# NVIDIA/k8s-operator-libs

Measured on AMD Instinct MI355X. Metric: 8-node rolling-upgrade wall-clock, lower is better.
Workload: dtype fp32; 1 GPU; model=amdgpu-driver-rolling-upgrade, nodes_per_cluster=8, maxParallelUpgrades=2, maxUnavailable=50%, drain=True, podDeletion=True, gpu_pods_per_node=2, gpu_validation=True, converging_reconcile=True, mode=inplace, global_batch=8, parallelism=dp1 (one independent simulated 8-node cluster per rank)

## Files before the change

### k8s_operator_libs_amd/core/cache.py

```python

from __future__ import annotations

import threading
import time
from typing import Dict, List, Optional, Tuple

from . import meta
from .client import Client
from .errors import NotFoundError
from .meta import K8sObject


class _Informer:
    BACKOFF_BASE = 0.1
    BACKOFF_MAX = 5.0

    USE_WATCH_LIST = True

    USE_DRAIN_ON_READ = True

    def __init__(self, delegate: Client, api_version: str, kind: str,
                 sync_delay: float = 0.0) -> None:
        self.api_version = api_version
        self.kind = kind
# ... 277 lines not shown
                self._informers[key] = inf
                inf.start()
        inf.wait_sync()
        return inf

    def wait_for_resource_version(self, api_version: str, kind: str,
                                  name: str, namespace: str, rv: str,
                                  timeout: float = 10.0) -> bool:
        return self._informer_for(api_version, kind).wait_for_rv(
            name, namespace, rv, timeout
        )

    def wait_for_cache_sync(self, timeout: float = 10.0) -> bool:
        with self._lock:
            informers = list(self._informers.values())
        return all(inf.wait_sync(timeout) for inf in informers)

    def stop(self) -> None:
        with self._lock:
            informers = list(self._informers.values())
            self._informers.clear()
        for inf in informers:
            inf.stop()


    def get(self, api_version, kind, name, namespace=""):
        return self._informer_for(api_version, kind).get(name, namespace)

    def list(self, api_version, kind, namespace=None, label_selector="", field_selector=""):
        return self._informer_for(api_version, kind).list(
            namespace, label_selector, field_selector
        )


    def create(self, obj):
        return self._delegate.create(obj)

    def update(self, obj):
        return self._delegate.update(obj)

    def patch(self, api_version, kind, name, patch, namespace=""):
        return self._delegate.patch(api_version, kind, name, patch, namespace)

    def delete(self, api_version, kind, name, namespace="", grace_period_seconds=None):
        try:
            self._delegate.delete(api_version, kind, name, namespace,
                                  grace_period_seconds=grace_period_seconds)
        except TypeError:
            self._delegate.delete(api_version, kind, name, namespace)

    def evict_pod(self, name, namespace):
        self._delegate.evict_pod(name, namespace)

    def patch_status(self, api_version, kind, name, status, namespace=""):
        return self._delegate.patch_status(api_version, kind, name, status,
                                           namespace)

    def watch(self, api_version, kind, namespace=None, resource_version=None,
              label_selector=""):
        return self._delegate.watch(
            api_version, kind, namespace=namespace,
            resource_version=resource_version, label_selector=label_selector,
        )

    def list_with_meta(self, api_version, kind, namespace=None,
                       label_selector="", field_selector=""):
        return self._delegate.list_with_meta(
            api_version, kind, namespace=namespace,
            label_selector=label_selector, field_selector=field_selector,
        )
```

### k8s_operator_libs_amd/core/client.py

```python

from __future__ import annotations

import abc
from typing import List, Optional

from .fakecluster import FakeCluster, Watch
from .meta import K8sObject


class Client(abc.ABC):

    @abc.abstractmethod
    def get(self, api_version: str, kind: str, name: str, namespace: str = "") -> K8sObject: ...

    @abc.abstractmethod
    def list(
        self,
        api_version: str,
        kind: str,
        namespace: Optional[str] = None,
        label_selector: str = "",
        field_selector: str = "",
    ) -> List[K8sObject]: ...

    @abc.abstractmethod
    def create(self, obj: K8sObject) -> K8sObject: ...

    @abc.abstractmethod
    def update(self, obj: K8sObject) -> K8sObject: ...

    @abc.abstractmethod
    def patch(
        self, api_version: str, kind: str, name: str, patch: K8sObject, namespace: str = ""
    ) -> K8sObject: ...

    @abc.abstractmethod
    def delete(self, api_version: str, kind: str, name: str, namespace: str = "") -> None:
        """Delete an object.  Implementations may accept a
        ``grace_period_seconds`` keyword (pod graceful-deletion override);
        in-memory substrates delete immediately and ignore it."""

    @abc.abstractmethod
    def evict_pod(self, name: str, namespace: str) -> None: ...

    def watch(
        self,
        api_version: str,
        kind: str,
        namespace: Optional[str] = None,
        resource_version: Optional[str] = None,
        label_selector: str = "",
    ) -> Watch:
        raise NotImplementedError("this client does not support watches")

    def list_with_meta(
        self,
        api_version: str,
        kind: str,
        namespace: Optional[str] = None,
        label_selector: str = "",
# ... 99 lines not shown
```

### k8s_operator_libs_amd/core/restclient.py

```python

from __future__ import annotations

import collections
import http.client as _http_client
import json
import os
from typing import Any, Dict, Optional

import httpx

from ..native import load_wire as _load_wire
from . import meta
from .client import Client
from .errors import (
    AlreadyExistsError,
    ApiError,
    BadRequestError,
    ConflictError,
    NotFoundError,
)

SA_DIR = "/var/run/secrets/kubernetes.io/serviceaccount"

_KIND_INFO = {
    ("v1", "Node"): ("nodes", False),
    ("v1", "Pod"): ("pods", True),
    ("v1", "Event"): ("events", True),
    ("v1", "Namespace"): ("namespaces", False),
    ("apps/v1", "DaemonSet"): ("daemonsets", True),
    ("apps/v1", "ControllerRevision"): ("controllerrevisions", True),
    ("apiextensions.k8s.io/v1", "CustomResourceDefinition"): (
        "customresourcedefinitions", False),
    ("maintenance.amd.com/v1alpha1", "NodeMaintenance"): ("nodemaintenances", True),
    ("coordination.k8s.io/v1", "Lease"): ("leases", True),
}


def _lower_plural(kind: str) -> str:
    k = kind.lower()
    if k.endswith(("ss", "x", "z", "ch", "sh")):
        return k + "es"
    if k.endswith("s"):
        return k
    if k.endswith("y") and len(k) > 1 and k[-2] not in "aeiou":
        return k[:-1] + "ies"
    return k + "s"


def _pool_max_idle() -> int:
    from ..upgrade.common_manager import CommonUpgradeManager
    from ..upgrade.drain_manager import DrainManager
    from ..upgrade.pod_manager import PodManager

    return (1 + PodManager.MAX_CONCURRENT_NODE_WORKERS
            + DrainManager.MAX_CONCURRENT_NODE_WORKERS
            + CommonUpgradeManager.MAX_PARALLEL_NODE_OPS)


class RestClient(Client):
    USE_POOL = True

    def __init__(
        self,
        base_url: str,
        token: Optional[str] = None,
        verify: Any = True,
        timeout: float = 30.0,
        extra_kinds: Optional[Dict[tuple, tuple]] = None,
        retries: int = 3,
    ) -> None:
        self.base_url = base_url.rstrip("/")
        headers = {"Content-Type": "application/json"}
        if token:
            headers["Authorization"] = f"Bearer {token}"
        self._headers = dict(headers)
        self._timeout = timeout
        self._http = httpx.Client(
            base_url=self.base_url, headers=headers, verify=verify, timeout=timeout
        )
        self._fast_netloc = None
        self._wire = None
        self._pool = None
        if self.base_url.startswith("http://"):
            import urllib.parse

            parsed = urllib.parse.urlsplit(self.base_url)
            self._fast_netloc = (parsed.hostname, parsed.port or 80)
            self._fast_local = __import__("threading").local()
            self._wire = _load_wire()
            self._wire_heads: Dict[tuple, bytes] = {}
            if self._wire is not None and hasattr(self._wire, "Pool"):
                self._pool = self._wire.Pool(
                    *self._fast_netloc, max_idle=_pool_max_idle(),
                    connect_timeout=timeout)
        self._kinds = dict(_KIND_INFO)
        if extra_kinds:
            self._kinds.update(extra_kinds)
        self._retries = retries


    def _wire_head(self, headers=None) -> bytes:
        key = tuple(sorted(headers.items())) if headers else ()
        head = self._wire_heads.get(key)
        if head is None:
            host, port = self._fast_netloc
            if ":" in host:
                host = f"[{host}]"
            hdrs = {"Host": host if port == 80 else f"{host}:{port}",
                    "Accept-Encoding": "identity"}
            hdrs.update(self._headers)
            if headers:
                hdrs.update(headers)
            head = "".join(f"{k}: {v}\r\n" for k, v in hdrs.items()).encode(
# ... 275 lines not shown
            md = body.get("metadata") or {}
            if rv is None:
                rv = md.get("resourceVersion")
            items.extend(body.get("items", []))
            cont = md.get("continue")
            if not cont:
                return items, rv
            params["continue"] = cont

    def create(self, obj):
        api_version, kind = meta.api_version(obj), meta.kind(obj)
        path = self._collection_path(api_version, kind, meta.namespace(obj))
        resp = self._request("POST", path, content=json.dumps(obj))
        self._raise_for(resp)
        return resp.json()

    def update(self, obj):
        api_version, kind = meta.api_version(obj), meta.kind(obj)
        path = self._object_path(api_version, kind, meta.name(obj), meta.namespace(obj))
        resp = self._request("PUT", path, content=json.dumps(obj))
        self._raise_for(resp)
        return resp.json()

    def patch(self, api_version, kind, name, patch, namespace=""):
        path = self._object_path(api_version, kind, name, namespace)
        resp = self._request(
            "PATCH", path, content=json.dumps(patch),
            headers={"Content-Type": "application/merge-patch+json"},
        )
        self._raise_for(resp)
        return resp.json()

    def delete(self, api_version, kind, name, namespace="", grace_period_seconds=None):
        kw = {}
        if grace_period_seconds is not None:
            kw["content"] = json.dumps({
                "apiVersion": "v1", "kind": "DeleteOptions",
                "gracePeriodSeconds": int(grace_period_seconds),
            })
        resp = self._request(
            "DELETE", self._object_path(api_version, kind, name, namespace), **kw
        )
        self._raise_for(resp)

    def patch_status(self, api_version, kind, name, status, namespace=""):
        path = self._object_path(api_version, kind, name, namespace) + "/status"
        resp = self._request(
            "PATCH", path, content=json.dumps({"status": status}),
            headers={"Content-Type": "application/merge-patch+json"},
        )
        self._raise_for(resp)
        return resp.json()

    def evict_pod(self, name, namespace):
        path = self._object_path("v1", "Pod", name, namespace) + "/eviction"
        body = {
            "apiVersion": "policy/v1",
            "kind": "Eviction",
            "metadata": {"name": name, "namespace": namespace},
        }
        resp = self._request("POST", path, content=json.dumps(body))
        self._raise_for(resp)

    def watch(self, api_version: str, kind: str, namespace=None,
              resource_version=None, label_selector="", field_selector="",
              send_initial_events=False):
        return _HttpWatch(self, api_version, kind, namespace=namespace,
                          resource_version=resource_version,
                          label_selector=label_selector,
                          field_selector=field_selector,
                          send_initial_events=send_initial_events)


    def discover_resource(self, api_version: str, plural: str) -> bool:
        prefix = f"/api/{api_version}" if "/" not in api_version else f"/apis/{api_version}"
        resp = self._request("GET", prefix)
        if resp.status_code != 200:
            return False
        for res in resp.json().get("resources", []):
            if res.get("name") == plural:
                return True
        return False

    def register_kind(self, api_version: str, kind: str, plural: str, namespaced: bool) -> None:
        self._kinds[(api_version, kind)] = (plural, namespaced)

    def close(self) -> None:
        self._http.close()
        if self._fast_netloc is not None:
            conn = getattr(self._fast_local, "conn", None)
            if conn is not None:
                try:
                    conn.close()
                except Exception:
                    pass
                self._fast_local.conn = None
            self._wire_drop(getattr(self._fast_local, "sock", None))
            pool, self._pool = self._pool, None
            if pool is not None:
                pool.close()


class _PoolClosed(Exception):
    """The client was closed while a request was on its way to the pool."""


class _FastResponse:

    __slots__ = ("status_code", "_data")

    def __init__(self, status_code: int, data: bytes) -> None:
        self.status_code = status_code
        self._data = data

    def json(self):
# ... 309 lines not shown
```

### k8s_operator_libs_amd/native/build.py

```python

from __future__ import annotations

import os
import subprocess
import sysconfig

PKG_DIR = os.path.dirname(os.path.abspath(__file__))
SOURCE = os.path.join(PKG_DIR, "gpu_validator.hip")
OUTPUT = os.path.join(PKG_DIR, "_gpu_validator.so")
JSONOPS_SOURCE = os.path.join(PKG_DIR, "jsonops.cpp")
JSONOPS_OUTPUT = os.path.join(PKG_DIR, "_jsonops.so")
WIRE_SOURCES = (
    os.path.join(PKG_DIR, "wire.cpp"),
    os.path.join(PKG_DIR, "wire_core.hpp"),
    os.path.join(PKG_DIR, "wire_pool.hpp"),
    os.path.join(PKG_DIR, "wire_stream.hpp"),
)
WIRE_OUTPUT = os.path.join(PKG_DIR, "_wire.so")

HIPCC = os.environ.get("HIPCC", "/opt/rocm/bin/hipcc")
CXX = os.environ.get("CXX", "g++")


def validator_sources() -> list:
    wire = {os.path.basename(p) for p in WIRE_SOURCES}
    return [SOURCE] + sorted(
        os.path.join(PKG_DIR, name) for name in os.listdir(PKG_DIR)
        if name.endswith(".hpp") and name not in wire)


def is_built() -> bool:
    return os.path.exists(OUTPUT) and all(
        os.path.getmtime(OUTPUT) >= os.path.getmtime(src)
        for src in validator_sources())


def build_jsonops(force: bool = False, verbose: bool = False) -> str:
    if (
        not force
        and os.path.exists(JSONOPS_OUTPUT)
        and os.path.getmtime(JSONOPS_OUTPUT) >= os.path.getmtime(JSONOPS_SOURCE)
    ):
        return JSONOPS_OUTPUT
    cmd = [
        CXX, "-O3", "-std=c++17", "-fPIC", "-shared",
        f"-I{sysconfig.get_paths()['include']}",
        JSONOPS_SOURCE, "-o", JSONOPS_OUTPUT,
    ]
    if verbose:
        print(" ".join(cmd))
    subprocess.run(cmd, check=True, capture_output=not verbose)
    return JSONOPS_OUTPUT


def build_wire(force: bool = False, verbose: bool = False) -> str:
    if (
        not force
        and os.path.exists(WIRE_OUTPUT)
        and all(os.path.getmtime(WIRE_OUTPUT) >= os.path.getmtime(src)
                for src in WIRE_SOURCES)
    ):
        return WIRE_OUTPUT
    cmd = [
        CXX, "-O3", "-std=c++17", "-fPIC", "-shared", "-pthread",
        f"-I{sysconfig.get_paths()['include']}",
        WIRE_SOURCES[0], "-o", WIRE_OUTPUT,
    ]
# ... 36 lines not shown
```

### k8s_operator_libs_amd/native/wire.cpp

```cpp

#define PY_SSIZE_T_CLEAN
#include <Python.h>

#include <atomic>
#include <cerrno>
#include <chrono>
#include <memory>
#include <mutex>
#include <new>
#include <string>
#include <system_error>
#include <thread>
#include <vector>

#include <fcntl.h>
#include <poll.h>
#include <sys/socket.h>
#include <sys/types.h>
#include <unistd.h>

#include "wire_core.hpp"
#include "wire_pool.hpp"
#include "wire_stream.hpp"

namespace {

constexpr size_t kRecvBuf = 64 * 1024;

using Clock = std::chrono::steady_clock;

struct Deadline {
  bool infinite;
  Clock::time_point at;

  explicit Deadline(double timeout_s) : infinite(timeout_s < 0) {
    if (!infinite)
      at = Clock::now() + std::chrono::duration_cast<Clock::duration>(
                              std::chrono::duration<double>(timeout_s));
  }

  int remaining_ms() const {
    if (infinite) return -1;
    auto left = std::chrono::duration_cast<std::chrono::microseconds>(
                    at - Clock::now()).count();
    if (left <= 0) return 0;
    long long ms = (left + 999) / 1000;
    return ms > 0x7fffffff ? 0x7fffffff : int(ms);
  }
};

bool parse_timeout(PyObject* obj, double* out) {
  if (obj == nullptr || obj == Py_None) {
    *out = -1.0;
    return true;
  }
  double v = PyFloat_AsDouble(obj);
  if (v == -1.0 && PyErr_Occurred()) return false;
  *out = v < 0 ? 0.0 : v;
  return true;
}

enum IoResult { kIoOk = 0, kIoTimeout = 1, kIoError = 2, kIoSignal = 3 };

IoResult wait_fd(int fd, short events, const Deadline& dl) {
  for (;;) {
    int ms = dl.remaining_ms();
    struct pollfd p = {fd, events, 0};
    int rc, err;
    Py_BEGIN_ALLOW_THREADS
    rc = poll(&p, 1, ms);
    err = errno;
    Py_END_ALLOW_THREADS
    if (rc > 0) return kIoOk;
    if (rc == 0) {
// ... 73 lines not shown
  return kIoOk;
}

PyObject* raise_wire_error(int st) {
  PyErr_SetString(PyExc_ValueError, wire::status_message(st));
  return nullptr;
}

PyObject* raise_timeout() {
  PyErr_SetString(PyExc_TimeoutError, "timed out");
  return nullptr;
}

bool as_buffer(PyObject* obj, const char** p, Py_ssize_t* n, bool* present) {
  *present = true;
  if (obj == Py_None) {
    *p = "";
    *n = 0;
    *present = false;
    return true;
  }
  if (PyBytes_Check(obj)) {
    *p = PyBytes_AS_STRING(obj);
    *n = PyBytes_GET_SIZE(obj);
    return true;
  }
  if (PyUnicode_Check(obj)) {
    *p = PyUnicode_AsUTF8AndSize(obj, n);
    return *p != nullptr;
  }
  PyErr_SetString(PyExc_TypeError, "body must be bytes, str or None");
  return false;
}


PyObject* py_exchange(PyObject* , PyObject* args) {
  int fd;
  const char *method, *path, *head;
  Py_ssize_t method_len, path_len, head_len;
  PyObject *body_obj, *timeout_obj = Py_None;
  if (!PyArg_ParseTuple(args, "is#s#y#O|O", &fd, &method, &method_len, &path,
                        &path_len, &head, &head_len, &body_obj, &timeout_obj))
    return nullptr;
  const char* body;
  Py_ssize_t body_len;
  bool has_body;
  if (!as_buffer(body_obj, &body, &body_len, &has_body)) return nullptr;
  double timeout_s;
  if (!parse_timeout(timeout_obj, &timeout_s)) return nullptr;
  Deadline dl(timeout_s);

  std::string method_s(method, size_t(method_len));
  bool is_head = method_s == "HEAD";
  bool wants_length = has_body || method_s == "POST" || method_s == "PUT" ||
                      method_s == "PATCH";

  std::string req;
  req.reserve(size_t(method_len + path_len + head_len + body_len) + 64);
  req.append(method_s).append(" ").append(path, size_t(path_len));
  req.append(" HTTP/1.1\r\n").append(head, size_t(head_len));
  if (wants_length)
    req.append("Content-Length: ").append(std::to_string(body_len)).append("\r\n");
  req.append("\r\n").append(body, size_t(body_len));

  IoResult io = send_all(fd, req.data(), req.size(), dl);
  if (io == kIoTimeout) return raise_timeout();
  if (io != kIoOk) return nullptr;

  wire::ResponseReader reader(is_head);
  char buf[kRecvBuf];

  while (!reader.done()) {
    size_t got = 0;
    io = recv_some(fd, buf, sizeof buf, dl, &got);
    if (io == kIoTimeout) return raise_timeout();
    if (io != kIoOk) return nullptr;
    if (got == 0) {
      if (reader.peer_closed()) break;
      bool got_any = reader.started();
      PyErr_SetString(got_any ? PyExc_ConnectionError
                              : PyExc_ConnectionResetError,
                      got_any ? "peer closed the connection mid-response"
                              : "peer closed the connection without a response");
      return nullptr;
    }
    int st = reader.feed(buf, got);
    if (st < 0) return raise_wire_error(st);
  }

  const std::string& out = reader.body();
  PyObject* body_bytes =
      PyBytes_FromStringAndSize(out.data(), Py_ssize_t(out.size()));
  if (!body_bytes) return nullptr;
  PyObject* res = Py_BuildValue("(iNO)", reader.status(), body_bytes,
                                reader.reusable() ? Py_True : Py_False);
  return res;
}


PyObject* py_parse_request_head(PyObject* , PyObject* arg) {
  Py_buffer view;
  if (PyObject_GetBuffer(arg, &view, PyBUF_SIMPLE) < 0) return nullptr;
  wire::HeadParser hp(wire::HeadParser::kRequest);
  size_t used = 0;
  int st = hp.feed(static_cast<const char*>(view.buf), size_t(view.len), &used);
  PyBuffer_Release(&view);
  if (st < 0) return raise_wire_error(st);
  if (st == wire::kNeedMore) Py_RETURN_NONE;
  PyObject* length;
  if (hp.has_content_length) {
    length = PyLong_FromSize_t(hp.content_length);
    if (!length) return nullptr;
  } else {
    length = Py_None;
    Py_INCREF(length);
  }
// ... 783 lines not shown
  switch (lease.error) {
    case wire::Pool::kOk:
      return Py_BuildValue("(iO)", lease.fd,
                           lease.reused ? Py_True : Py_False);
    case wire::Pool::kClosed:
      PyErr_SetString(PyExc_RuntimeError, "Pool is closed");
      return nullptr;
    case wire::Pool::kResolve: {
      PyObject* gaierror = nullptr;
      PyObject* mod = PyImport_ImportModule("socket");
      if (mod != nullptr) {
        gaierror = PyObject_GetAttrString(mod, "gaierror");
        Py_DECREF(mod);
      }
      if (gaierror == nullptr) return nullptr;
      PyObject* val = Py_BuildValue("(is)", lease.code, gai_strerror(lease.code));
      if (val != nullptr) {
        PyErr_SetObject(gaierror, val);
        Py_DECREF(val);
      }
      Py_DECREF(gaierror);
      return nullptr;
    }
    case wire::Pool::kTimeout:
      return raise_timeout();
    case wire::Pool::kInterrupted:
      return nullptr;
    default:
      errno = lease.code;
      return PyErr_SetFromErrno(PyExc_OSError);
  }
}

PyObject* pool_checkout(PoolObject* self, PyObject* args) {
  try {
    return pool_checkout_impl(self, args);
  } catch (const std::bad_alloc&) {
    return PyErr_NoMemory();
  }
}

PyObject* pool_checkin(PoolObject* self, PyObject* args) {
  int fd, reusable;
  if (!PyArg_ParseTuple(args, "ip", &fd, &reusable)) return nullptr;
  if (!pool_enter(self)) return nullptr;
  try {
    self->pool->checkin(fd, reusable != 0);
  } catch (const std::bad_alloc&) {
    close(fd);
  }
  Py_RETURN_NONE;
}

PyObject* pool_close(PoolObject* self, PyObject*) {
  if (!pool_enter(self)) return nullptr;
  self->pool->close();
  Py_RETURN_NONE;
}

PyObject* pool_stats(PoolObject* self, PyObject*) {
  if (!pool_enter(self)) return nullptr;
  wire::PoolStats st = self->pool->stats();
  return Py_BuildValue("{s:K,s:K,s:K,s:n}", "dials",
                       static_cast<unsigned long long>(st.dials), "reuses",
                       static_cast<unsigned long long>(st.reuses),
                       "stale_discards",
                       static_cast<unsigned long long>(st.stale_discards),
                       "idle", Py_ssize_t(st.idle));
}

PyObject* pool_get_max_idle(PoolObject* self, void*) {
  if (!pool_enter(self)) return nullptr;
  return PyLong_FromSize_t(self->pool->max_idle());
}

PyObject* pool_get_closed(PoolObject* self, void*) {
  if (!pool_enter(self)) return nullptr;
  return PyBool_FromLong(self->pool->closed());
}

PyMethodDef pool_methods[] = {
    {"checkout", reinterpret_cast<PyCFunction>(pool_checkout), METH_VARARGS,
     "checkout(fresh=False) -> (fd, reused).  The most recently used idle "
     "connection that is still quiet (reused=True), else (or with fresh) a "
     "new one, dialled with the GIL released.  The fd stays the pool's: pass it to exchange() and "
     "give it back with checkin(), exactly once, never close it.  OSError "
     "(TimeoutError, socket.gaierror) when the dial fails; RuntimeError "
     "once the pool is closed."},
    {"checkin", reinterpret_cast<PyCFunction>(pool_checkin), METH_VARARGS,
     "checkin(fd, reusable).  Give a checked-out fd back.  It is kept for "
     "the next checkout() only when reusable is true (the response was "
     "complete and exchange() said reusable), the pool is open and fewer "
     "than max_idle are idle; otherwise the pool closes it."},
    {"close", reinterpret_cast<PyCFunction>(pool_close), METH_NOARGS,
     "close().  Close the idle connections; one checked out now is closed "
     "when it comes back.  checkout() raises from here on."},
    {"stats", reinterpret_cast<PyCFunction>(pool_stats), METH_NOARGS,
     "stats() -> {'dials', 'reuses', 'stale_discards', 'idle'}."},
    {nullptr, nullptr, 0, nullptr},
};

PyGetSetDef pool_getset[] = {
    {"max_idle", reinterpret_cast<getter>(pool_get_max_idle), nullptr,
     "most connections kept idle", nullptr},
    {"closed", reinterpret_cast<getter>(pool_get_closed), nullptr,
     "True after close()", nullptr},
    {nullptr, nullptr, nullptr, nullptr, nullptr},
};

PyTypeObject PoolType = {
    PyVarObject_HEAD_INIT(nullptr, 0)
    "_wire.Pool",
    sizeof(PoolObject),
};


PyObject* py_exchange_guarded(PyObject* self, PyObject* args) {
  try {
    return py_exchange(self, args);
  } catch (const std::bad_alloc&) {
    return PyErr_NoMemory();
  }
}

PyObject* py_parse_request_head_guarded(PyObject* self, PyObject* arg) {
  try {
    return py_parse_request_head(self, arg);
  } catch (const std::bad_alloc&) {
    return PyErr_NoMemory();
  }
}

PyMethodDef wire_methods[] = {
    {"exchange", py_exchange_guarded, METH_VARARGS,
     "exchange(fd, method, path, header_bytes, body, timeout=None) -> "
     "(status, body_bytes, reusable).  One HTTP/1.1 request/response on a "
     "connected socket: the request goes out in a single send; the response "
     "is read with Content-Length, chunked or read-to-EOF framing.  "
     "reusable is False when the connection must not carry another request."},
    {"parse_request_head", py_parse_request_head_guarded, METH_O,
     "parse_request_head(data) -> None | (method, target, minor_version, "
     "content_length | None, chunked, keep_alive, head_size).  None while "
     "the head is incomplete; ValueError when it is malformed."},
    {nullptr, nullptr, 0, nullptr},
};

// ... 93 lines not shown
```

### k8s_operator_libs_amd/upgrade/drain.py

```python

from __future__ import annotations

import logging
import time
from dataclasses import dataclass, field
from typing import Callable, List, Optional

from ..api.upgrade.v1alpha1 import DrainSpec
from ..core import meta
from ..core.client import Client
from ..core.errors import ApiError, NotFoundError
from . import consts

logger = logging.getLogger(__name__)

MIRROR_POD_ANNOTATION = "kubernetes.io/config.mirror"

PodFilter = Callable[[dict], bool]


@dataclass
class PodDeleteList:

    pods: List[dict] = field(default_factory=list)
# ... 49 lines not shown
    node_name: str,
    *,
    force: bool = False,
    delete_emptydir_data: bool = False,
    ignore_daemonsets: bool = True,
    pod_selector: str = "",
    additional_filter: Optional[PodFilter] = None,
) -> PodDeleteList:
    pods = client.list_pods(
        label_selector=pod_selector,
        field_selector=consts.NODE_NAME_FIELD_SELECTOR_FMT.format(node_name),
    )
    out = PodDeleteList()
    for pod in pods:
        pname = f"{meta.namespace(pod)}/{meta.name(pod)}"
        if _is_terminating(pod):
            out.skipped.append(pod)
            continue
        if additional_filter is not None and not additional_filter(pod):
            out.skipped.append(pod)
            continue
        if _is_mirror_pod(pod):
            out.skipped.append(pod)
            out.warnings.append(f"skipping mirror pod {pname}")
            continue
        if _is_daemonset_pod(pod):
            if ignore_daemonsets:
                out.skipped.append(pod)
                out.warnings.append(f"ignoring DaemonSet-managed pod {pname}")
                continue
            out.errors.append(f"cannot delete DaemonSet-managed pod {pname}")
            continue
        if _is_finished(pod):
            out.pods.append(pod)
            continue
        if not _has_controller(pod) and not force:
            out.errors.append(
                f"cannot delete pod not managed by a controller (use force): {pname}"
            )
            continue
        if _uses_emptydir(pod) and not delete_emptydir_data:
            out.errors.append(
                f"cannot delete pod with emptyDir volume (use deleteEmptyDir): {pname}"
            )
            continue
        out.pods.append(pod)
    return out


class DrainError(Exception):
    pass


def delete_or_evict_pods(
    client: Client,
    pods: List[dict],
    *,
    use_eviction: bool = True,
    timeout_seconds: float = 300,
) -> None:
    deadline = time.monotonic() + max(timeout_seconds, 0.001)

    def try_evict(pod) -> bool:
        try:
            if use_eviction:
                client.evict_pod(meta.name(pod), meta.namespace(pod))
            else:
                client.delete_pod(meta.name(pod), meta.namespace(pod))
            return True
        except NotFoundError:
            return True
        except ApiError as exc:
            if exc.code == 429:
                return False
            raise

    blocked = [pod for pod in pods if not try_evict(pod)]
    interval = 0.001
    remaining = list(pods)
    while remaining:
        blocked = [pod for pod in blocked if not try_evict(pod)]
        still_there = []
        for pod in remaining:
            try:
                live = client.get("v1", "Pod", meta.name(pod), meta.namespace(pod))
            except NotFoundError:
                continue
            if meta.uid(live) == meta.uid(pod):
                still_there.append(pod)
        remaining = still_there
        if not remaining:
            return
        if time.monotonic() >= deadline:
            names = [f"{meta.namespace(p)}/{meta.name(p)}" for p in remaining]
            if blocked:
                names = [f"{n} (PDB-blocked)" if any(
                    meta.name(b) == n.split("/")[-1] for b in blocked) else n
                    for n in names]
            raise DrainError(f"timed out waiting for pods to terminate: {names}")
        time.sleep(interval)
        interval = min(interval * 2, 0.5)


def drain_node(client: Client, node_name: str, spec: DrainSpec) -> None:
    plist = get_pods_for_deletion(
        client,
        node_name,
        force=spec.force,
        delete_emptydir_data=spec.delete_emptydir_data,
        ignore_daemonsets=True,
        pod_selector=spec.pod_selector,
    )
    if plist.errors:
        raise DrainError("; ".join(plist.errors))
    for warning in plist.warnings:
        logger.debug("drain %s: %s", node_name, warning)
    delete_or_evict_pods(
        client, plist.pods, use_eviction=True, timeout_seconds=spec.timeout_seconds
    )
```

### k8s_operator_libs_amd/upgrade/pod_manager.py

```python

from __future__ import annotations

import logging
import threading
import time
from dataclasses import dataclass, field
from typing import Callable, List, Optional

from ..api.upgrade.v1alpha1 import PodDeletionSpec, WaitForCompletionSpec
from ..core import meta
from ..core.client import Client
from ..core.events import EVENT_TYPE_NORMAL, EVENT_TYPE_WARNING, log_event, log_eventf
from ..core.meta import K8sObject
from . import consts, util
from .drain import delete_or_evict_pods, get_pods_for_deletion
from .node_state_provider import NodeUpgradeStateProvider

logger = logging.getLogger(__name__)

class StaleClusterViewError(RuntimeError):
    """The client's view is missing objects that must exist (e.g. a managed
    DaemonSet with no ControllerRevisions): with an informer-backed client
    this is a transient staleness window, not a cluster defect.  Callers
    treat it like any reconcile error — requeue (upgrade_state.go:128-131
    pattern)."""


POD_CONTROLLER_REVISION_HASH_LABEL = "controller-revision-hash"

PodDeletionFilter = Callable[[K8sObject], bool]


@dataclass
class PodManagerConfig:

    nodes: List[K8sObject] = field(default_factory=list)
    deletion_spec: Optional[PodDeletionSpec] = None
    wait_for_completion_spec: Optional[WaitForCompletionSpec] = None
    drain_enabled: bool = False


class PodManager:
    def __init__(
        self,
        client: Client,
        node_state_provider: NodeUpgradeStateProvider,
        pod_deletion_filter: Optional[PodDeletionFilter] = None,
        event_recorder: Optional[object] = None,
    ) -> None:
        self._client = client
        self._provider = node_state_provider
        self._filter = pod_deletion_filter
        self._recorder = event_recorder
        self._nodes_in_progress = util.StringSet()
        self._workers: List[threading.Thread] = []
        self._workers_lock = threading.Lock()
        self._worker_slots = threading.Semaphore(self.MAX_CONCURRENT_NODE_WORKERS)
        self._ds_hash_cache: dict = {}


    def get_pod_controller_revision_hash(self, pod: K8sObject) -> str:
        hash_ = meta.get_label(pod, POD_CONTROLLER_REVISION_HASH_LABEL)
        if not hash_:
            raise ValueError(
                f"pod {meta.name(pod)} has no {POD_CONTROLLER_REVISION_HASH_LABEL} label"
            )
        return hash_

    def get_daemonset_controller_revision_hash(self, daemonset: K8sObject) -> str:
        cache_key = (meta.namespace(daemonset), meta.name(daemonset),
                     meta.resource_version(daemonset))
        cached = self._ds_hash_cache.get(cache_key)
        if cached is not None:
            return cached
        selector = daemonset.get("spec", {}).get("selector", {}).get("matchLabels", {})
        label_selector = ",".join(f"{k}={v}" for k, v in sorted(selector.items()))
        revisions = self._client.list_controller_revisions(
            namespace=meta.namespace(daemonset), label_selector=label_selector
        )
        if not revisions:
            raise StaleClusterViewError(
                f"no ControllerRevisions found for DaemonSet {meta.name(daemonset)}"
            )
        latest = max(revisions, key=lambda r: r.get("revision", 0))
        prefix = f"{meta.name(daemonset)}-"
        name = meta.name(latest)
        hash_ = name[len(prefix):] if name.startswith(prefix) else name
        if len(self._ds_hash_cache) > 256:
            self._ds_hash_cache.clear()
        self._ds_hash_cache[cache_key] = hash_
        return hash_


    def schedule_pod_eviction(self, config: PodManagerConfig) -> None:
        if not config.nodes:
            logger.info("no nodes scheduled for pod deletion")
            return
        if config.deletion_spec is None:
            raise ValueError("pod deletion spec should not be empty")
        for node in config.nodes:
            node_name = meta.name(node)
            if not self._nodes_in_progress.add_if_absent(node_name):
                logger.info("node %s already getting pods deleted, skipping", node_name)
                continue
            self._spawn(self._evict_node_worker, node, config)

    def _evict_node_worker(self, node: K8sObject, config: PodManagerConfig) -> None:
        node_name = meta.name(node)
        spec = config.deletion_spec
        try:
            pods = self._client.list_pods(
                field_selector=consts.NODE_NAME_FIELD_SELECTOR_FMT.format(node_name)
            )
            to_delete = [p for p in pods if self._filter and self._filter(p)]
            if not to_delete:
                logger.info("no pods require deletion on node %s", node_name)
                self._provider.change_node_upgrade_state(
                    node, consts.UPGRADE_STATE_POD_RESTART_REQUIRED
                )
                return
            plist = get_pods_for_deletion(
                self._client,
                node_name,
                force=spec.force,
                delete_emptydir_data=spec.delete_emptydir_data,
                ignore_daemonsets=True,
                additional_filter=self._filter,
            )
            if len(plist.pods) != len(to_delete):
                logger.error(
                    "cannot delete all required pods on node %s: %s",
                    node_name, plist.errors,
                )
                self._update_node_to_drain_or_failed(node, config.drain_enabled)
                return
            try:
                delete_or_evict_pods(
                    self._client, plist.pods,
                    use_eviction=True, timeout_seconds=spec.timeout_seconds,
                )
            except Exception as exc:
                log_eventf(
                    self._recorder, node, EVENT_TYPE_WARNING, util.get_event_reason(),
                    "Failed to delete workload pods on the node for the driver upgrade, {}",
                    exc,
                )
                self._update_node_to_drain_or_failed(node, config.drain_enabled)
                return
            self._provider.change_node_upgrade_state(
                node, consts.UPGRADE_STATE_POD_RESTART_REQUIRED
            )
            log_event(self._recorder, node, EVENT_TYPE_NORMAL, util.get_event_reason(),
                      "Deleted workload pods on the node for the driver upgrade")
        except Exception:
            logger.exception("pod eviction worker failed for node %s", node_name)
        finally:
            self._nodes_in_progress.remove(node_name)

    def _update_node_to_drain_or_failed(self, node: K8sObject, drain_enabled: bool) -> None:
        next_state = consts.UPGRADE_STATE_FAILED
        if drain_enabled:
            log_event(self._recorder, node, EVENT_TYPE_WARNING, util.get_event_reason(),
                      "Pod deletion failed but drain is enabled in spec. Will attempt a node drain")
            next_state = consts.UPGRADE_STATE_DRAIN_REQUIRED
        self._provider.change_node_upgrade_state(node, next_state)


    def schedule_pods_restart(self, pods: List[K8sObject]) -> None:
        if not pods:
            logger.info("no pods scheduled to restart")
            return
        for pod in pods:
            logger.info("deleting driver pod %s for restart", meta.name(pod))
            try:
                self._client.delete_pod(meta.name(pod), meta.namespace(pod))
            except Exception as exc:
                log_eventf(self._recorder, pod, EVENT_TYPE_WARNING, util.get_event_reason(),
                           "Failed to restart driver pod {}", exc)
                raise


    def schedule_check_on_pod_completion(self, config: PodManagerConfig) -> None:
        spec = config.wait_for_completion_spec or WaitForCompletionSpec()
        threads = []
        for node in config.nodes:
            t = threading.Thread(
                target=self._completion_check_worker, args=(node, spec), daemon=True
            )
            t.start()
            threads.append(t)
        for t in threads:
            t.join()

    def _completion_check_worker(self, node: K8sObject, spec: WaitForCompletionSpec) -> None:
        node_name = meta.name(node)
        try:
            pods = self._client.list_pods(
                label_selector=spec.pod_selector,
                field_selector=consts.NODE_NAME_FIELD_SELECTOR_FMT.format(node_name),
            )
            running = any(self.is_pod_running_or_pending(p) for p in pods)
            if running:
                logger.info("workload pods still running on node %s", node_name)
                if spec.timeout_seconds != 0:
                    self.handle_timeout_on_pod_completions(node, spec.timeout_seconds)
                return
# ... 54 lines not shown
```

Before: 24.50 ms.

## Batch pod evictions across nodes through native pipelined exchange_many

Adds a native exchange_many to the wire pool. It sends many HTTP requests at once and polls all of them from one thread with the GIL released. The pod manager now gathers every pod to evict on the scheduled nodes, evicts them in one batched call inline, and confirms the pods are gone with a short cache catch-up wait. It falls back to per-node worker threads only when some pod was not cleanly evicted. This removes thread spawning and serial eviction round trips, but adds a large new C++ polling path with resend and error-mapping logic, and runs the eviction synchronously in the reconcile caller.

```diff
diff --git a/k8s_operator_libs_amd/core/cache.py b/k8s_operator_libs_amd/core/cache.py
--- a/k8s_operator_libs_amd/core/cache.py
+++ b/k8s_operator_libs_amd/core/cache.py
@@ -353,6 +353,13 @@
     def evict_pod(self, name, namespace):
         self._delegate.evict_pod(name, namespace)
 
+    @property
+    def supports_batch_eviction(self) -> bool:
+        return bool(getattr(self._delegate, "supports_batch_eviction", False))
+
+    def evict_pods(self, pods, max_in_flight: int = 0) -> list:
+        return self._delegate.evict_pods(pods, max_in_flight=max_in_flight)
+
     def patch_status(self, api_version, kind, name, status, namespace=""):
         return self._delegate.patch_status(api_version, kind, name, status,
                                            namespace)
diff --git a/k8s_operator_libs_amd/core/client.py b/k8s_operator_libs_amd/core/client.py
--- a/k8s_operator_libs_amd/core/client.py
+++ b/k8s_operator_libs_amd/core/client.py
@@ -6,6 +6,9 @@
 
 from .fakecluster import FakeCluster, Watch
 from .meta import K8sObject
+
+EVICTION_ACCEPTED = "accepted"
+EVICTION_BLOCKED = "blocked"
 
 
 class Client(abc.ABC):
diff --git a/k8s_operator_libs_amd/core/restclient.py b/k8s_operator_libs_amd/core/restclient.py
--- a/k8s_operator_libs_amd/core/restclient.py
+++ b/k8s_operator_libs_amd/core/restclient.py
@@ -11,7 +11,7 @@
 
 from ..native import load_wire as _load_wire
 from . import meta
-from .client import Client
+from .client import EVICTION_ACCEPTED, EVICTION_BLOCKED, Client
 from .errors import (
     AlreadyExistsError,
     ApiError,
@@ -59,6 +59,8 @@
 
 class RestClient(Client):
     USE_POOL = True
+
+    USE_EXCHANGE_MANY = True
 
     def __init__(
         self,
@@ -440,15 +442,69 @@
         self._raise_for(resp)
         return resp.json()
 
-    def evict_pod(self, name, namespace):
+    def _eviction_request(self, name, namespace) -> tuple:
         path = self._object_path("v1", "Pod", name, namespace) + "/eviction"
         body = {
             "apiVersion": "policy/v1",
             "kind": "Eviction",
             "metadata": {"name": name, "namespace": namespace},
         }
-        resp = self._request("POST", path, content=json.dumps(body))
+        return path, json.dumps(body)
+
+    def evict_pod(self, name, namespace):
+        path, body = self._eviction_request(name, namespace)
+        resp = self._request("POST", path, content=body)
         self._raise_for(resp)
+
+    @property
+    def supports_batch_eviction(self) -> bool:
+        pool = self._pool
+        return bool(self.USE_EXCHANGE_MANY and self.USE_POOL
+                    and pool is not None and hasattr(pool, "exchange_many"))
+
+    def evict_pods(self, pods, max_in_flight: int = 0) -> list:
+        if not self.supports_batch_eviction:
+            raise RuntimeError("batch eviction needs the native wire pool "
+                               "(see supports_batch_eviction)")
+        head = self._wire_head()
+        requests = []
+        for pod in pods:
+            path, body = self._eviction_request(meta.name(pod),
+                                                meta.namespace(pod))
+            requests.append(("POST", path, head, body))
+        try:
+            results = self._pool.exchange_many(requests, self._timeout,
+                                               max_in_flight)
+        except RuntimeError as exc:
+            results = [exc] * len(requests)
+        outcomes = []
+        for pod, result in zip(pods, results):
+            if isinstance(result, BaseException) or \
+                    result[0] in (500, 502, 503, 504):
+                outcomes.append(self._evict_pod_outcome(pod))
+            else:
+                outcomes.append(self._eviction_outcome(_FastResponse(*result)))
+        return outcomes
+
+    def _evict_pod_outcome(self, pod):
+        try:
+            self.evict_pod(meta.name(pod), meta.namespace(pod))
+        except NotFoundError:
+            pass
+        except ApiError as exc:
+            return EVICTION_BLOCKED if exc.code == 429 else exc
+        return EVICTION_ACCEPTED
+
+    def _eviction_outcome(self, resp):
+        if resp.status_code < 400 or resp.status_code == 404:
+            return EVICTION_ACCEPTED
+        if resp.status_code == 429:
+            return EVICTION_BLOCKED
+        try:
+            self._raise_for(resp)
+        except ApiError as exc:
+            return exc
+        raise AssertionError("unreachable")
 
     def watch(self, api_version: str, kind: str, namespace=None,
               resource_version=None, label_selector="", field_selector="",
diff --git a/k8s_operator_libs_amd/native/build.py b/k8s_operator_libs_amd/native/build.py
--- a/k8s_operator_libs_amd/native/build.py
+++ b/k8s_operator_libs_amd/native/build.py
@@ -13,6 +13,7 @@
 WIRE_SOURCES = (
     os.path.join(PKG_DIR, "wire.cpp"),
     os.path.join(PKG_DIR, "wire_core.hpp"),
+    os.path.join(PKG_DIR, "wire_many.hpp"),
     os.path.join(PKG_DIR, "wire_pool.hpp"),
     os.path.join(PKG_DIR, "wire_stream.hpp"),
 )
diff --git a/k8s_operator_libs_amd/native/wire.cpp b/k8s_operator_libs_amd/native/wire.cpp
--- a/k8s_operator_libs_amd/native/wire.cpp
+++ b/k8s_operator_libs_amd/native/wire.cpp
@@ -20,6 +20,7 @@
 #include <unistd.h>
 
 #include "wire_core.hpp"
+#include "wire_many.hpp"
 #include "wire_pool.hpp"
 #include "wire_stream.hpp"
 
@@ -199,16 +200,10 @@
 
   std::string method_s(method, size_t(method_len));
   bool is_head = method_s == "HEAD";
-  bool wants_length = has_body || method_s == "POST" || method_s == "PUT" ||
-                      method_s == "PATCH";
-
-  std::string req;
-  req.reserve(size_t(method_len + path_len + head_len + body_len) + 64);
-  req.append(method_s).append(" ").append(path, size_t(path_len));
-  req.append(" HTTP/1.1\r\n").append(head, size_t(head_len));
-  if (wants_length)
-    req.append("Content-Length: ").append(std::to_string(body_len)).append("\r\n");
-  req.append("\r\n").append(body, size_t(body_len));
+
+  std::string req = wire::assemble_request(
+      method_s, path, size_t(path_len), head, size_t(head_len), body,
+      size_t(body_len), has_body);
 
   IoResult io = send_all(fd, req.data(), req.size(), dl);
   if (io == kIoTimeout) return raise_timeout();
@@ -1098,6 +1093,139 @@
   Py_RETURN_NONE;
 }
 
+PyObject* new_gaierror(int code) {
+  PyObject* mod = PyImport_ImportModule("socket");
+  if (mod == nullptr) return nullptr;
+  PyObject* gaierror = PyObject_GetAttrString(mod, "gaierror");
+  Py_DECREF(mod);
+  if (gaierror == nullptr) return nullptr;
+  PyObject* exc = PyObject_CallFunction(gaierror, "is", code, gai_strerror(code));
+  Py_DECREF(gaierror);
+  return exc;
+}
+
+PyObject* many_entry(const wire::ManyResult& r) {
+  switch (r.kind) {
+    case wire::ManyResult::kResponse: {
+      PyObject* body =
+          PyBytes_FromStringAndSize(r.body.data(), Py_ssize_t(r.body.size()));
+      if (!body) return nullptr;
+      return Py_BuildValue("(iN)", r.status, body);
+    }
+    case wire::ManyResult::kTimeout:
+      return PyObject_CallFunction(PyExc_TimeoutError, "s", "timed out");
+    case wire::ManyResult::kResolve:
+      return new_gaierror(r.code);
+    case wire::ManyResult::kNoResponse:
+      return PyObject_CallFunction(
+          PyExc_ConnectionResetError, "s",
+          "peer closed the connection without a response");
+    case wire::ManyResult::kCutShort:
+      return PyObject_CallFunction(PyExc_ConnectionError, "s",
+                                   "peer closed the connection mid-response");
+    case wire::ManyResult::kFraming:
+      return PyObject_CallFunction(PyExc_ValueError, "s",
+                                   wire::status_message(r.code));
+    default:
+      return PyObject_CallFunction(PyExc_OSError, "is", r.code,
+                                   std::strerror(r.code));
+  }
+}
+
+PyObject* pool_exchange_many_impl(PoolObject* self, PyObject* args,
+                                  PyObject* kw) {
+  static const char* names[] = {"requests", "timeout", "max_in_flight",
+                                nullptr};
+  PyObject* requests_obj;
+  PyObject* timeout_obj = Py_None;
+  Py_ssize_t max_in_flight = 0;
+  if (!PyArg_ParseTupleAndKeywords(args, kw, "O|On", const_cast<char**>(names),
+                                   &requests_obj, &timeout_obj,
+                                   &max_in_flight))
+    return nullptr;
+  if (!pool_enter(self)) return nullptr;
+  if (max_in_flight < 0) {
+    PyErr_SetString(PyExc_ValueError, "max_in_flight must be >= 0");
+    return nullptr;
+  }
+  double timeout_s;
+  if (!parse_timeout(timeout_obj, &timeout_s)) return nullptr;
+  PyObject* seq = PySequence_Fast(
+      requests_obj, "requests must be a sequence of (method, path, "
+                    "header_bytes, body) tuples");
+  if (seq == nullptr) return nullptr;
+  std::vector<wire::ManyRequest> requests(size_t(PySequence_Fast_GET_SIZE(seq)));
+  for (size_t i = 0; i < requests.size(); ++i) {
+    PyObject* item = PySequence_Fast_GET_ITEM(seq, Py_ssize_t(i));
+    const char *method, *path, *head;
+    Py_ssize_t method_len, path_len, head_len;
+    PyObject* body_obj;
+    const char* body;
+    Py_ssize_t body_len;
+    bool has_body;
+    if (!PyTuple_Check(item)) {
+      PyErr_SetString(PyExc_TypeError,
+                      "each request must be a (method, path, header_bytes, "
+                      "body) tuple");
+      Py_DECREF(seq);
+      return nullptr;
+    }
+    if (!PyArg_ParseTuple(item, "s#s#y#O", &method, &method_len, &path,
+                          &path_len, &head, &head_len, &body_obj) ||
+        !as_buffer(body_obj, &body, &body_len, &has_body)) {
+      Py_DECREF(seq);
+      return nullptr;
+    }
+    std::string method_s(method, size_t(method_len));
+    requests[i].is_head = method_s == "HEAD";
+    requests[i].bytes = wire::assemble_request(
+        method_s, path, size_t(path_len), head, size_t(head_len), body,
+        size_t(body_len), has_body);
+  }
+  Py_DECREF(seq);
+
+  std::vector<wire::ManyResult> results;
+  wire::ManyOutcome outcome;
+  bool no_memory = false;
+  Py_BEGIN_ALLOW_THREADS
+  try {
+    outcome = wire::exchange_many(*self->pool, requests, timeout_s,
+                                  size_t(max_in_flight), &results,
+                                  pool_on_eintr, nullptr);
+  } catch (const std::bad_alloc&) {
+    no_memory = true;
+    outcome = wire::kManyClosed;
+  }
+  Py_END_ALLOW_THREADS
+  if (no_memory) return PyErr_NoMemory();
+  if (outcome == wire::kManyClosed) {
+    PyErr_SetString(PyExc_RuntimeError, "Pool is closed");
+    return nullptr;
+  }
+  if (outcome == wire::kManyInterrupted)
+    return nullptr;
+
+  PyObject* out = PyList_New(Py_ssize_t(results.size()));
+  if (!out) return nullptr;
+  for (size_t i = 0; i < results.size(); ++i) {
+    PyObject* entry = many_entry(results[i]);
+    if (!entry) {
+      Py_DECREF(out);
+      return nullptr;
+    }
+    PyList_SET_ITEM(out, Py_ssize_t(i), entry);
+  }
+  return out;
+}
+
+PyObject* pool_exchange_many(PoolObject* self, PyObject* args, PyObject* kw) {
+  try {
+    return pool_exchange_many_impl(self, args, kw);
+  } catch (const std::bad_alloc&) {
+    return PyErr_NoMemory();
+  }
+}
+
 PyObject* pool_close(PoolObject* self, PyObject*) {
   if (!pool_enter(self)) return nullptr;
   self->pool->close();
@@ -1138,6 +1266,23 @@
      "the next checkout() only when reusable is true (the response was "
      "complete and exchange() said reusable), the pool is open and fewer "
      "than max_idle are idle; otherwise the pool closes it."},
+    {"exchange_many", reinterpret_cast<PyCFunction>(pool_exchange_many),
+     METH_VARARGS | METH_KEYWORDS,
+     "exchange_many(requests, timeout=None, max_in_flight=0) -> list.  "
+     "requests: a sequence of (method, path, header_bytes, body | None), "
+     "the pieces exchange() takes.  One entry per request, in request "
+     "order: (status, body_bytes), or the exception instance (OSError, "
+     "TimeoutError, ValueError for malformed framing) that request alone "
+     "ran into; those are returned, not raised.  The calling thread does "
+     "everything, the GIL released throughout: a lease per request, one "
+     "send each, poll() over all of them, every fd checked back in and "
+     "kept only after a complete reusable response.  max_in_flight (0: "
+     "max_idle) bounds the connections in use; the surplus is written as "
+     "they free up.  timeout is per request, from the moment it is "
+     "written.  A request is sent again, once, on a fresh dial, only when "
+     "its idle-list connection was reset or closed before any byte of a "
+     "response.  Raises for bad arguments, RuntimeError once the pool is "
+     "closed, or what a signal handler raised; every lease is closed first."},
     {"close", reinterpret_cast<PyCFunction>(pool_close), METH_NOARGS,
      "close().  Close the idle connections; one checked out now is closed "
      "when it comes back.  checkout() raises from here on."},
diff --git a/k8s_operator_libs_amd/native/wire_many.hpp b/k8s_operator_libs_amd/native/wire_many.hpp
--- /dev/null
+++ b/k8s_operator_libs_amd/native/wire_many.hpp
@@ -0,0 +1,323 @@
+
+#pragma once
+
+#include <cerrno>
+#include <chrono>
+#include <cstddef>
+#include <new>
+#include <string>
+#include <vector>
+
+#include <poll.h>
+#include <sys/socket.h>
+#include <sys/types.h>
+
+#include "wire_core.hpp"
+#include "wire_pool.hpp"
+
+namespace wire {
+
+inline std::string assemble_request(const std::string& method,
+                                    const char* path, size_t path_len,
+                                    const char* head, size_t head_len,
+                                    const char* body, size_t body_len,
+                                    bool has_body) {
+  bool wants_length = has_body || method == "POST" || method == "PUT" ||
+                      method == "PATCH";
+  std::string req;
+  req.reserve(method.size() + path_len + head_len + body_len + 64);
+  req.append(method).append(" ").append(path, path_len);
+  req.append(" HTTP/1.1\r\n").append(head, head_len);
+  if (wants_length)
+    req.append("Content-Length: ").append(std::to_string(body_len)).append("\r\n");
+  req.append("\r\n").append(body, body_len);
+  return req;
+}
+
+struct ManyRequest {
+  std::string bytes;
+  bool is_head = false;
+};
+
+struct ManyResult {
+  enum Kind {
+    kPending = 0,
+    kResponse,
+    kTimeout,
+    kOsError,
+    kResolve,
+    kNoResponse,
+    kCutShort,
+    kFraming,
+  };
+  Kind kind = kPending;
+  int status = 0;
+  int code = 0;
+  std::string body;
+};
+
+struct ManyCounters {
+  size_t leases = 0;
+  size_t checkins = 0;
+  size_t resends = 0;
+};
+
+enum ManyOutcome { kManyOk = 0, kManyClosed, kManyInterrupted };
+
+namespace detail {
+
+using ManyClock = std::chrono::steady_clock;
+
+struct ManySlot {
+  explicit ManySlot(size_t index_, bool is_head)
+      : index(index_), reader(is_head) {}
+
+  size_t index;
+  int fd = -1;
+  bool reused = false;
+  bool resent = false;
+  size_t sent = 0;
+  bool infinite = true;
+  ManyClock::time_point deadline;
+  ResponseReader reader;
+};
+
+inline bool is_reset(int err) {
+  return err == ECONNRESET || err == EPIPE;
+}
+
+}
+
+inline ManyOutcome exchange_many(Pool& pool,
+                                 const std::vector<ManyRequest>& requests,
+                                 double timeout_s, size_t max_in_flight,
+                                 std::vector<ManyResult>* out,
+                                 Pool::OnEintr on_eintr = nullptr,
+                                 void* arg = nullptr,
+                                 ManyCounters* counters = nullptr) {
+  using detail::ManyClock;
+  using detail::ManySlot;
+  ManyCounters local;
+  ManyCounters& count = counters ? *counters : local;
+  count = ManyCounters();
+  if (max_in_flight == 0) max_in_flight = pool.max_idle();
+  if (max_in_flight == 0) max_in_flight = 1;
+  out->clear();
+  if (pool.closed()) return kManyClosed;
+  out->resize(requests.size());
+
+  std::vector<ManySlot> active;
+  active.reserve(max_in_flight < requests.size() ? max_in_flight
+                                                 : requests.size());
+  std::vector<struct pollfd> fds;
+  std::vector<char> buf(64 * 1024);
+  size_t next = 0;
+
+  auto give_back = [&](ManySlot& s, bool reusable) {
+    if (s.fd < 0) return;
+    int fd = s.fd;
+    s.fd = -1;
+    ++count.checkins;
+    try {
+      pool.checkin(fd, reusable);
+    } catch (const std::bad_alloc&) {
+      ::close(fd);
+      throw;
+    }
+  };
+  struct CloseLeases {
+    std::vector<ManySlot>& slots;
+    Pool& pool;
+    ManyCounters& count;
+    ~CloseLeases() {
+      for (ManySlot& s : slots) {
+        if (s.fd < 0) continue;
+        ++count.checkins;
+        pool.checkin(s.fd, false);
+      }
+    }
+  } close_leases{active, pool, count};
+  auto abort_all = [&](ManyOutcome why) {
+    for (ManySlot& s : active) give_back(s, false);
+    active.clear();
+    out->clear();
+    return why;
+  };
+  auto finish = [&](ManySlot& s, ManyResult::Kind kind, int code,
+                    bool reusable) {
+    ManyResult& r = (*out)[s.index];
+    r.kind = kind;
+    r.code = code;
+    if (kind == ManyResult::kResponse) {
+      r.status = s.reader.status();
+      r.body.swap(s.reader.body());
+    }
+    give_back(s, reusable);
+  };
+
+  auto lease_slot = [&](ManySlot& s, bool fresh) -> ManyOutcome {
+    Pool::Lease lease = fresh ? pool.dial(on_eintr, arg)
+                              : pool.checkout(on_eintr, arg);
+    if (lease.fd < 0) {
+      switch (lease.error) {
+        case Pool::kClosed: return kManyClosed;
+        case Pool::kInterrupted: return kManyInterrupted;
+        case Pool::kTimeout: finish(s, ManyResult::kTimeout, 0, false); break;
+        case Pool::kResolve:
+          finish(s, ManyResult::kResolve, lease.code, false);
+          break;
+        default: finish(s, ManyResult::kOsError, lease.code, false); break;
+      }
+      return kManyOk;
+    }
+    ++count.leases;
+    s.fd = lease.fd;
+    s.reused = lease.reused;
+    s.sent = 0;
+    s.infinite = timeout_s < 0;
+    if (!s.infinite)
+      s.deadline = ManyClock::now() +
+                   std::chrono::duration_cast<ManyClock::duration>(
+                       std::chrono::duration<double>(timeout_s));
+    return kManyOk;
+  };
+
+  auto resend = [&](ManySlot& s, ManyOutcome* stop) -> bool {
+    if (!s.reused || s.resent || s.reader.started()) return false;
+    give_back(s, false);
+    s.resent = true;
+    ++count.resends;
+    *stop = lease_slot(s, true);
+    return true;
+  };
+
+  auto write_some = [&](ManySlot& s, ManyOutcome* stop) -> bool {
+    for (;;) {
+      if (s.fd < 0) return false;
+      const std::string& req = requests[s.index].bytes;
+      if (s.sent == req.size()) return true;
+      ssize_t n = send(s.fd, req.data() + s.sent, req.size() - s.sent,
+                       MSG_NOSIGNAL | MSG_DONTWAIT);
+      if (n >= 0) {
+        s.sent += size_t(n);
+        continue;
+      }
+      int err = errno;
+      if (err == EINTR) continue;
+      if (err == EAGAIN || err == EWOULDBLOCK) return true;
+      if (detail::is_reset(err) && resend(s, stop)) {
+        if (*stop != kManyOk) return false;
+        continue;
+      }
+      finish(s, ManyResult::kOsError, err, false);
+      return false;
+    }
+  };
+
+  auto read_some = [&](ManySlot& s, ManyOutcome* stop) -> bool {
+    for (;;) {
+      ssize_t n = recv(s.fd, buf.data(), buf.size(), MSG_DONTWAIT);
+      if (n > 0) {
+        int st = s.reader.feed(buf.data(), size_t(n));
+        if (st < 0) {
+          finish(s, ManyResult::kFraming, st, false);
+          return false;
+        }
+        if (s.reader.done()) {
+          finish(s, ManyResult::kResponse, 0, s.reader.reusable());
+          return false;
+        }
+        continue;
+      }
+      int err = errno;
+      if (n < 0) {
+        if (err == EINTR) continue;
+        if (err == EAGAIN || err == EWOULDBLOCK) return true;
+        if (!detail::is_reset(err)) {
+          finish(s, ManyResult::kOsError, err, false);
+          return false;
+        }
+      } else if (s.reader.peer_closed()) {
+        finish(s, ManyResult::kResponse, 0, false);
+        return false;
+      }
+      if (resend(s, stop)) {
+        if (*stop != kManyOk) return false;
+        return write_some(s, stop);
+      }
+      if (n < 0)
+        finish(s, ManyResult::kOsError, err, false);
+      else
+        finish(s, s.reader.started() ? ManyResult::kCutShort
+                                     : ManyResult::kNoResponse, 0, false);
+      return false;
+    }
+  };
+
+  while (next < requests.size() || !active.empty()) {
+    while (active.size() < max_in_flight && next < requests.size()) {
+      active.emplace_back(next, requests[next].is_head);
+      ++next;
+      ManyOutcome stop = lease_slot(active.back(), false);
+      if (stop != kManyOk) return abort_all(stop);
+      if (active.back().fd < 0 || !write_some(active.back(), &stop)) {
+        if (stop != kManyOk) return abort_all(stop);
+        active.pop_back();
+      }
+    }
+    if (active.empty()) continue;
+
+    fds.clear();
+    int wait_ms = -1;
+    ManyClock::time_point now = ManyClock::now();
+    for (ManySlot& s : active) {
+      bool writing = s.sent < requests[s.index].bytes.size();
+      fds.push_back({s.fd, short(writing ? POLLOUT : POLLIN), 0});
+      if (s.infinite) continue;
+      auto left = std::chrono::duration_cast<std::chrono::microseconds>(
+                      s.deadline - now).count();
+      long long ms = left <= 0 ? 0 : (left + 999) / 1000;
+      if (ms > 0x7fffffff) ms = 0x7fffffff;
+      if (wait_ms < 0 || ms < wait_ms) wait_ms = int(ms);
+    }
+    int rc = poll(fds.data(), nfds_t(fds.size()), wait_ms);
+    if (rc < 0) {
+      int err = errno;
+      if (err == EINTR) {
+        if (on_eintr && !on_eintr(arg)) return abort_all(kManyInterrupted);
+        continue;
+      }
+      for (ManySlot& s : active) finish(s, ManyResult::kOsError, err, false);
+      active.clear();
+      continue;
+    }
+
+    now = ManyClock::now();
+    size_t kept = 0;
+    for (size_t i = 0; i < active.size(); ++i) {
+      ManySlot& s = active[i];
+      bool alive = true;
+      ManyOutcome stop = kManyOk;
+      if (fds[i].revents != 0) {
+        bool writing = s.sent < requests[s.index].bytes.size();
+        if (writing) alive = write_some(s, &stop);
+        if (alive && s.sent == requests[s.index].bytes.size() &&
+            (!writing || (fds[i].revents & (POLLIN | POLLHUP | POLLERR))))
+          alive = read_some(s, &stop);
+        if (stop != kManyOk) return abort_all(stop);
+      }
+      if (alive && !s.infinite && now >= s.deadline) {
+        finish(s, ManyResult::kTimeout, 0, false);
+        alive = false;
+      }
+      if (alive) {
+        if (kept != i) active[kept] = std::move(s);
+        ++kept;
+      }
+    }
+    active.erase(active.begin() + long(kept), active.end());
+  }
+  return kManyOk;
+}
+
+}
diff --git a/k8s_operator_libs_amd/upgrade/drain.py b/k8s_operator_libs_amd/upgrade/drain.py
--- a/k8s_operator_libs_amd/upgrade/drain.py
+++ b/k8s_operator_libs_amd/upgrade/drain.py
@@ -125,14 +125,24 @@
     pass
 
 
+def pod_is_gone(client: Client, pod: dict) -> bool:
+    try:
+        live = client.get("v1", "Pod", meta.name(pod), meta.namespace(pod))
+    except NotFoundError:
+        return True
+    return meta.uid(live) != meta.uid(pod)
+
+
 def delete_or_evict_pods(
     client: Client,
     pods: List[dict],
     *,
     use_eviction: bool = True,
     timeout_seconds: float = 300,
+    already_accepted: Optional[List[dict]] = None,
 ) -> None:
     deadline = time.monotonic() + max(timeout_seconds, 0.001)
+    accepted = {id(pod) for pod in already_accepted or ()}
 
     def try_evict(pod) -> bool:
         try:
@@ -148,20 +158,13 @@
                 return False
             raise
 
-    blocked = [pod for pod in pods if not try_evict(pod)]
+    blocked = [pod for pod in pods
+               if id(pod) not in accepted and not try_evict(pod)]
     interval = 0.001
     remaining = list(pods)
     while remaining:
         blocked = [pod for pod in blocked if not try_evict(pod)]
-        still_there = []
-        for pod in remaining:
-            try:
-                live = client.get("v1", "Pod", meta.name(pod), meta.namespace(pod))
-            except NotFoundError:
-                continue
-            if meta.uid(live) == meta.uid(pod):
-                still_there.append(pod)
-        remaining = still_there
+        remaining = [pod for pod in remaining if not pod_is_gone(client, pod)]
         if not remaining:
             return
         if time.monotonic() >= deadline:
diff --git a/k8s_operator_libs_amd/upgrade/pod_manager.py b/k8s_operator_libs_amd/upgrade/pod_manager.py
--- a/k8s_operator_libs_amd/upgrade/pod_manager.py
+++ b/k8s_operator_libs_amd/upgrade/pod_manager.py
@@ -9,11 +9,11 @@
 
 from ..api.upgrade.v1alpha1 import PodDeletionSpec, WaitForCompletionSpec
 from ..core import meta
-from ..core.client import Client
+from ..core.client import EVICTION_ACCEPTED, Client
 from ..core.events import EVENT_TYPE_NORMAL, EVENT_TYPE_WARNING, log_event, log_eventf
 from ..core.meta import K8sObject
 from . import consts, util
-from .drain import delete_or_evict_pods, get_pods_for_deletion
+from .drain import delete_or_evict_pods, get_pods_for_deletion, pod_is_gone
 from .node_state_provider import NodeUpgradeStateProvider
 
 logger = logging.getLogger(__name__)
@@ -98,46 +98,137 @@
             return
         if config.deletion_spec is None:
             raise ValueError("pod deletion spec should not be empty")
+        nodes = []
         for node in config.nodes:
             node_name = meta.name(node)
             if not self._nodes_in_progress.add_if_absent(node_name):
                 logger.info("node %s already getting pods deleted, skipping", node_name)
                 continue
+            nodes.append(node)
+        if nodes and self.SYNC_EVICTION_FAST_PATH and getattr(
+                self._client, "supports_batch_eviction", False):
+            self._evict_nodes_inline(nodes, config)
+            return
+        for node in nodes:
             self._spawn(self._evict_node_worker, node, config)
 
-    def _evict_node_worker(self, node: K8sObject, config: PodManagerConfig) -> None:
+    SYNC_EVICTION_FAST_PATH = True
+
+    def _evict_nodes_inline(self, nodes: List[K8sObject],
+                            config: PodManagerConfig) -> None:
+        mine = {meta.name(node) for node in nodes}
+        try:
+            plans = []
+            for node in nodes:
+                try:
+                    pods = self._pods_to_evict(node, config)
+                except Exception:
+                    logger.exception("pod eviction failed for node %s",
+                                     meta.name(node))
+                    continue
+                if pods is not None:
+                    plans.append((node, pods))
+            if not plans:
+                return
+            outcomes = self._client.evict_pods(
+                [pod for _, pods in plans for pod in pods],
+                max_in_flight=len(plans) + 1)
+            at = 0
+            for node, pods in plans:
+                mine_out = outcomes[at:at + len(pods)]
+                at += len(pods)
+                done = all(o == EVICTION_ACCEPTED for o in mine_out) and all(
+                    self._gone_already(pod) for pod in pods)
+                if not done:
+                    mine.discard(meta.name(node))
+                    self._spawn(self._evict_node_worker, node, config,
+                                (pods, mine_out))
+                    continue
+                try:
+                    self._finish_eviction(node)
+                except Exception:
+                    logger.exception("pod eviction failed for node %s",
+                                     meta.name(node))
+        except Exception:
+            logger.exception("pod eviction failed for nodes %s", sorted(mine))
+        finally:
+            for node_name in mine:
+                self._nodes_in_progress.remove(node_name)
+
+    CACHE_CATCH_UP_SECONDS = 0.005
+
+    def _gone_already(self, pod: K8sObject) -> bool:
+        catch_up = getattr(self._client, "wait_for_resource_version", None)
+        if catch_up is not None:
+            try:
+                newer = str(int(meta.resource_version(pod)) + 1)
+            except (TypeError, ValueError):
+                newer = None
+            if newer is not None:
+                catch_up("v1", "Pod", meta.name(pod), meta.namespace(pod),
+                         newer, timeout=self.CACHE_CATCH_UP_SECONDS)
+        return pod_is_gone(self._client, pod)
+
+    def _pods_to_evict(self, node: K8sObject,
+                       config: PodManagerConfig) -> Optional[List[K8sObject]]:
+        node_name = meta.name(node)
+        spec = config.deletion_spec
+        pods = self._client.list_pods(
+            field_selector=consts.NODE_NAME_FIELD_SELECTOR_FMT.format(node_name)
+        )
+        to_delete = [p for p in pods if self._filter and self._filter(p)]
+        if not to_delete:
+            logger.info("no pods require deletion on node %s", node_name)
+            self._provider.change_node_upgrade_state(
+                node, consts.UPGRADE_STATE_POD_RESTART_REQUIRED
+            )
+            return None
+        plist = get_pods_for_deletion(
+            self._client,
+            node_name,
+            force=spec.force,
+            delete_emptydir_data=spec.delete_emptydir_data,
+            ignore_daemonsets=True,
+            additional_filter=self._filter,
+        )
+        if len(plist.pods) != len(to_delete):
+            logger.error(
+                "cannot delete all required pods on node %s: %s",
+                node_name, plist.errors,
+            )
+            self._update_node_to_drain_or_failed(node, config.drain_enabled)
+            return None
+        return plist.pods
+
+    def _finish_eviction(self, node: K8sObject) -> None:
+        self._provider.change_node_upgrade_state(
+            node, consts.UPGRADE_STATE_POD_RESTART_REQUIRED
+        )
+        log_event(self._recorder, node, EVENT_TYPE_NORMAL, util.get_event_reason(),
+                  "Deleted workload pods on the node for the driver upgrade")
+
+    def _evict_node_worker(self, node: K8sObject, config: PodManagerConfig,
+                           started=None) -> None:
         node_name = meta.name(node)
         spec = config.deletion_spec
         try:
-            pods = self._client.list_pods(
-                field_selector=consts.NODE_NAME_FIELD_SELECTOR_FMT.format(node_name)
-            )
-            to_delete = [p for p in pods if self._filter and self._filter(p)]
-            if not to_delete:
-                logger.info("no pods require deletion on node %s", node_name)
-                self._provider.change_node_upgrade_state(
-                    node, consts.UPGRADE_STATE_POD_RESTART_REQUIRED
-                )
-                return
-            plist = get_pods_for_deletion(
-                self._client,
-                node_name,
-                force=spec.force,
-                delete_emptydir_data=spec.delete_emptydir_data,
-                ignore_daemonsets=True,
-                additional_filter=self._filter,
-            )
-            if len(plist.pods) != len(to_delete):
-                logger.error(
-                    "cannot delete all required pods on node %s: %s",
-                    node_name, plist.errors,
-                )
-                self._update_node_to_drain_or_failed(node, config.drain_enabled)
-                return
+            accepted = None
+            if started is None:
+                pods = self._pods_to_evict(node, config)
+                if pods is None:
+                    return
+            else:
+                pods, outcomes = started
+                accepted = [pod for pod, outcome in zip(pods, outcomes)
+                            if outcome == EVICTION_ACCEPTED]
             try:
+                for outcome in outcomes if started is not None else ():
+                    if isinstance(outcome, Exception):
+                        raise outcome
                 delete_or_evict_pods(
-                    self._client, plist.pods,
+                    self._client, pods,
                     use_eviction=True, timeout_seconds=spec.timeout_seconds,
+                    already_accepted=accepted,
                 )
             except Exception as exc:
                 log_eventf(
@@ -147,11 +238,7 @@
                 )
                 self._update_node_to_drain_or_failed(node, config.drain_enabled)
                 return
-            self._provider.change_node_upgrade_state(
-                node, consts.UPGRADE_STATE_POD_RESTART_REQUIRED
-            )
-            log_event(self._recorder, node, EVENT_TYPE_NORMAL, util.get_event_reason(),
-                      "Deleted workload pods on the node for the driver upgrade")
+            self._finish_eviction(node)
         except Exception:
             logger.exception("pod eviction worker failed for node %s", node_name)
         finally:
```

Result: faster. 13.93 ms, median of 6 (-43.1%).
